# megaease/easevoice-trainer

Measured on AMD Instinct MI355X. Metric: audio-seconds/sec trained (s2), higher is better.
Workload: dtype bf16; 1 GPU; s2 SoVITS generator+discriminator GAN step, batch=16/GPU, 4 s 32 kHz clips (T=200 frames), configs/s2.json, random-init weights; global_batch=16, parallelism=dp1, launch=hip-graph replay (3 graphs/step)

## Files before the change

### easevoice_trainer_amd/csrc/elementwise.hip

```cpp
#include "evt_common.h"
#include "../../include/evt.h"

namespace {

__device__ __forceinline__ void store_w(void* base, long idx, float w, int dtype) {
  if (dtype == EVT_DT_HALF) reinterpret_cast<h16_t*>(base)[idx] = f2h(w);
  else reinterpret_cast<float*>(base)[idx] = w;
}

__device__ __forceinline__ long reg_idx(const evt_wlayout& L, int d0, int d1, int kk) {
  const int chunk = d1 / L.reg_ck, cc = d1 - chunk * L.reg_ck;
  return (((long)d0 * L.reg_nchunk + chunk) * L.reg_kp + kk) * L.reg_ck + cc;
}

__device__ __forceinline__ long alt_idx(const evt_wlayout& L, int d0, int d1, int kk) {
  const int chunk = d0 / L.alt_ck, cc = d0 - chunk * L.alt_ck;
  if (L.stride == 1) {
    const int t = L.k - 1 - kk;
    return (((long)d1 * L.alt_nchunk + chunk) * L.alt_kp + t) * L.alt_ck + cc;
  }
  const int J = (L.k + L.stride - 1) / L.stride;
  const int ph = kk % L.stride, j = kk / L.stride;
  const int jp = J - 1 - j;
  return ((((long)ph * L.d1 + d1) * L.alt_nchunk + chunk) * L.alt_kp + jp) * L.alt_ck + cc;
// ... 360 lines not shown

constexpr int SEG_MAX = 64;

template <typename T, int MODE>
__device__ __forceinline__ float seg_term(float a, float b, float target) {
  if (MODE == 0) return fabsf(a - b);
  const float d = target - a;
  return d * d;
}
template <typename T, int MODE>
__device__ __forceinline__ float seg_grad(float a, float b, float target, float dl) {
  if (MODE == 0) { const float d = a - b; return d > 0.f ? dl : (d < 0.f ? -dl : 0.f); }
  return -2.f * (target - a) * dl;
}

template <typename T, int MODE, bool BWD>
__global__ __launch_bounds__(256) void seg_flat_kernel(const evt_seg* segs, int nseg, float target, float* out,
                                                       const float* dloss) {
  constexpr int V = 16 / sizeof(T);
  __shared__ float red[4];
  __shared__ long pre[SEG_MAX + 1];
  if (threadIdx.x == 0) {
    long acc = 0;
    for (int i = 0; i < nseg; ++i) { pre[i] = acc; acc += segs[i].n; }
    pre[nseg] = acc;
  }
  __syncthreads();
  const long total = pre[nseg];
  long chunk = (total + gridDim.x - 1) / gridDim.x;
  chunk = (chunk + 2047) / 2048 * 2048;
  const long lo = (long)blockIdx.x * chunk, hi = min(total, lo + chunk);
  float acc = 0.f;
  for (int si = 0; si < nseg; ++si) {
    const long s0 = pre[si], s1 = pre[si + 1];
    if (s1 <= lo || s0 >= hi) continue;
    const evt_seg s = segs[si];
    if (BWD && !s.da) continue;
    const T* a = reinterpret_cast<const T*>(s.a);
    const T* b = reinterpret_cast<const T*>(s.b);
    T* da = reinterpret_cast<T*>(s.da);
    const long i0 = max(lo, s0) - s0, i1 = min(hi, s1) - s0;
    const float dl = BWD ? dloss[0] * s.scale : 0.f;
    float part = 0.f;
    const long v0 = min(i1, (i0 + V - 1) / V * V), v1 = v0 + (i1 - v0) / V * V;
    const bool vec_ok = ((((uintptr_t)a) | (MODE == 0 ? (uintptr_t)b : 0) | (BWD ? (uintptr_t)da : 0)) & 15) == 0;
    if (vec_ok) {
      for (long i = i0 + threadIdx.x; i < v0; i += 256) {
        const float av = to_f<T>(a[i]), bv = MODE == 0 ? to_f<T>(b[i]) : 0.f;
        if (BWD) da[i] = from_f<T>(seg_grad<T, MODE>(av, bv, target, dl)); else part += seg_term<T, MODE>(av, bv, target);
      }
      for (long i = v0 + (long)threadIdx.x * V; i < v1; i += 256L * V) {
        const uint4 va = *reinterpret_cast<const uint4*>(a + i);
        uint4 vb = make_uint4(0, 0, 0, 0);
        if (MODE == 0) vb = *reinterpret_cast<const uint4*>(b + i);
        const T* pa = reinterpret_cast<const T*>(&va);
        const T* pb = reinterpret_cast<const T*>(&vb);
        uint4 vo;
        T* po = reinterpret_cast<T*>(&vo);
#pragma unroll
        for (int e = 0; e < V; ++e) {
          const float av = to_f<T>(pa[e]), bv = MODE == 0 ? to_f<T>(pb[e]) : 0.f;
          if (BWD) po[e] = from_f<T>(seg_grad<T, MODE>(av, bv, target, dl)); else part += seg_term<T, MODE>(av, bv, target);
        }
        if (BWD) *reinterpret_cast<uint4*>(da + i) = vo;
      }
      for (long i = v1 + threadIdx.x; i < i1; i += 256) {
        const float av = to_f<T>(a[i]), bv = MODE == 0 ? to_f<T>(b[i]) : 0.f;
        if (BWD) da[i] = from_f<T>(seg_grad<T, MODE>(av, bv, target, dl)); else part += seg_term<T, MODE>(av, bv, target);
      }
    } else {
      for (long i = i0 + threadIdx.x; i < i1; i += 256) {
        const float av = to_f<T>(a[i]), bv = MODE == 0 ? to_f<T>(b[i]) : 0.f;
        if (BWD) da[i] = from_f<T>(seg_grad<T, MODE>(av, bv, target, dl)); else part += seg_term<T, MODE>(av, bv, target);
      }
    }
    acc += part * s.scale;
  }
  if (!BWD) {
    acc = block_reduce_sum_256(acc, red);
    if (threadIdx.x == 0 && acc != 0.f) atomicAdd(out, acc);
  }
}

__global__ void adamw_flat_kernel(float* p, const float* g, float* m, float* v, const evt_adamw_seg* segs, int nseg,
                                  float b1, float b2, float eps, float bc1, float bc2_sqrt, float gscale,
                                  long lo, long hi) {
  for (long i = lo + blockIdx.x * (long)blockDim.x + threadIdx.x; i < hi; i += (long)gridDim.x * blockDim.x) {
    int si = -1;
// ... 375 lines not shown
```

### easevoice_trainer_amd/csrc/losses.hip

```cpp
#include "evt_common.h"
#include "../../include/evt.h"

namespace {

__device__ __forceinline__ float ld_any(const void* p, int dt, long i) {
  return dt == EVT_DT_HALF ? h2f(reinterpret_cast<const h16_t*>(p)[i]) : reinterpret_cast<const float*>(p)[i];
}
__device__ __forceinline__ void st_any(void* p, int dt, long i, float v) {
  if (dt == EVT_DT_HALF) reinterpret_cast<h16_t*>(p)[i] = f2h(v); else reinterpret_cast<float*>(p)[i] = v;
}

struct KlArgs {
  const void* zp; const void* lq; const void* mp; const void* lp;
  void* dzp; void* dlq; void* dmp; void* dlp;
  int dt_zp, dt_lq, dt_mp, dt_lp;
  const int* lens;
  int B, T, C, time_inner;
};

__device__ __forceinline__ bool kl_live(const KlArgs& a, long i) {
  if (!a.lens) return true;
  long b, t;
  if (a.time_inner) { t = i % a.T; b = i / ((long)a.T * a.C); }
  else { const long row = i / a.C; b = row / a.T; t = row - b * a.T; }
  return t < a.lens[b];
}

__global__ __launch_bounds__(256) void masked_kl_fwd_kernel(KlArgs a, long n, float* out) {
  __shared__ float red[4];
  float acc = 0.f;
  for (long i = blockIdx.x * 256L + threadIdx.x; i < n; i += (long)gridDim.x * 256) {
    if (!kl_live(a, i)) continue;
    const float zp = ld_any(a.zp, a.dt_zp, i), lq = ld_any(a.lq, a.dt_lq, i), mp = ld_any(a.mp, a.dt_mp, i),
                lp = ld_any(a.lp, a.dt_lp, i);
    const float d = zp - mp;
    acc += lp - lq - 0.5f + 0.5f * d * d * __expf(-2.f * lp);
  }
  acc = block_reduce_sum_256(acc, red);
  if (threadIdx.x == 0) atomicAdd(out, acc);
  if (blockIdx.x == 0 && threadIdx.x == 0) {
    long cnt = 0;
    for (int b = 0; b < a.B; ++b) cnt += a.lens ? min(max(a.lens[b], 0), a.T) : a.T;
    out[1] = (float)cnt;
  }
}

__global__ __launch_bounds__(256) void masked_kl_bwd_kernel(KlArgs a, long n, const float* dloss, const float* count) {
  const float g = dloss[0] / count[0];
  for (long i = blockIdx.x * 256L + threadIdx.x; i < n; i += (long)gridDim.x * 256) {
    float gz = 0.f, glq = 0.f, glp = 0.f;
    if (kl_live(a, i)) {
      const float zp = ld_any(a.zp, a.dt_zp, i), mp = ld_any(a.mp, a.dt_mp, i), lp = ld_any(a.lp, a.dt_lp, i);
      const float d = zp - mp, e = __expf(-2.f * lp);
      gz = g * d * e;
      glq = -g;
      glp = g * (1.f - d * d * e);
    }
    if (a.dzp) st_any(a.dzp, a.dt_zp, i, gz);
    if (a.dlq) st_any(a.dlq, a.dt_lq, i, glq);
    if (a.dmp) st_any(a.dmp, a.dt_mp, i, -gz);
    if (a.dlp) st_any(a.dlp, a.dt_lp, i, glp);
  }
}

int kl_args(KlArgs& a, const evt_kl_params* p, const void* zp, const void* lq, const void* mp, const void* lp,
            const int32_t* lens) {
  if (!p || !zp || !lq || !mp || !lp || p->B <= 0 || p->T <= 0 || p->C <= 0) return EVT_EINVAL;
  const int dts[4] = {p->dt_z_p, p->dt_logs_q, p->dt_m_p, p->dt_logs_p};
  for (int d : dts) if (d != EVT_DT_F32 && d != EVT_DT_HALF) return EVT_EINVAL;
  a.zp = zp; a.lq = lq; a.mp = mp; a.lp = lp;
  a.dzp = a.dlq = a.dmp = a.dlp = nullptr;
  a.dt_zp = dts[0]; a.dt_lq = dts[1]; a.dt_mp = dts[2]; a.dt_lp = dts[3];
  a.lens = lens; a.B = p->B; a.T = p->T; a.C = p->C; a.time_inner = p->time_inner ? 1 : 0;
  return EVT_OK;
}

}

extern "C" {

int evt_masked_kl_fwd(const evt_kl_params* p, const void* z_p, const void* logs_q, const void* m_p, const void* logs_p,
                      const int32_t* lens, float* out2, void* stream) {
  KlArgs a;
  if (int rc = kl_args(a, p, z_p, logs_q, m_p, logs_p, lens)) return rc;
  if (!out2) return EVT_EINVAL;
  const long n = (long)p->B * p->T * p->C;
  long blocks = (n + 256L * 8 - 1) / (256L * 8);
  if (blocks > 2048) blocks = 2048;
  hipLaunchKernelGGL(masked_kl_fwd_kernel, dim3((unsigned)blocks), dim3(256), 0, (hipStream_t)stream, a, n, out2);
  return evt_check_launch();
}

int evt_masked_kl_bwd(const evt_kl_params* p, const void* z_p, const void* logs_q, const void* m_p, const void* logs_p,
                      const int32_t* lens, const float* dloss, const float* count, void* dz_p, void* dlogs_q, void* dm_p,
                      void* dlogs_p, void* stream) {
  KlArgs a;
  if (int rc = kl_args(a, p, z_p, logs_q, m_p, logs_p, lens)) return rc;
  if (!dloss || !count) return EVT_EINVAL;
  a.dzp = dz_p; a.dlq = dlogs_q; a.dmp = dm_p; a.dlp = dlogs_p;
  const long n = (long)p->B * p->T * p->C;
  long blocks = (n + 256L * 8 - 1) / (256L * 8);
  if (blocks > 2048) blocks = 2048;
  hipLaunchKernelGGL(masked_kl_bwd_kernel, dim3((unsigned)blocks), dim3(256), 0, (hipStream_t)stream, a, n, dloss, count);
  return evt_check_launch();
}

int64_t evt_workspace_bytes(int32_t op, const int64_t* dims, int32_t ndims) {
  if (!dims && ndims > 0) return -1;
  switch (op) {
    case EVT_WS_MEL:
      if (ndims != 5) return -1;
      return 4 * evt_mel_workspace_floats((int32_t)dims[0], (int32_t)dims[1], (int32_t)dims[2], (int32_t)dims[3],
                                          (int32_t)dims[4]);
    case EVT_WS_ATTN_BWD:
    case EVT_WS_MHA_BWD:
      if (ndims != 3) return -1;
      return 4 * dims[0] * dims[1] * dims[2];
    case EVT_WS_MASKED_KL:
// ... 10 lines not shown
```

### easevoice_trainer_amd/hip/disc.py

```python
import ctypes as C
import os

import torch

from . import conv as HC
from . import lib as L

_ALL = os.environ.get("EVT_BRANCH_STREAMS", "1") != "0"
MPD_STREAMS = int(os.environ.get("EVT_MPD_STREAMS", "2")) if _ALL else 1
_side = {}


def _new_stream(dev, k):
    return L.role_stream(dev, f"lane{k}", ring=1)


def _branches(dev, n_items):
    n = MPD_STREAMS if (dev.type == "cuda" and HC.TRACE is None) else 1
    if n <= 1:
        return [None] * n_items, []
    pool = _side.setdefault(dev, [])
    while len(pool) < n - 1:
        pool.append(_new_stream(dev, len(pool)))
    lanes = [None] + pool[: n - 1]
# ... 69 lines not shown
    @staticmethod
    def forward(ctx, x, periods, cd):
        ctx.periods, ctx.shape, ctx.dtype = periods, tuple(x.shape), x.dtype
        return tuple(mpd_fold(periods, cd, x))

    @staticmethod
    def backward(ctx, *grads):
        n, T = ctx.shape
        gs = []
        for g, p in zip(grads, ctx.periods):
            gs.append(g if g is not None else torch.zeros((n * p, (T + p - 1) // p, 1), dtype=grads[0].dtype,
                                                          device=grads[0].device))
        return mpd_unfold(ctx.periods, gs, 0, n, T, ctx.dtype), None, None


def _seg_table(a, b, da, scales, device):
    segs = [L.Seg(x.data_ptr(), y.data_ptr() if y is not None else None, g.data_ptr() if g is not None else None,
                  x.numel(), sc, 0) for x, y, g, sc in zip(a, b, da, scales)]
    return L.struct_to_device(segs, device)


class MPDGenLossFn(torch.autograd.Function):
    @staticmethod
    def forward(ctx, anchor, plan, periods, y_hat, y_real):
        nd = len(plan)
        n_items, T = y_hat.shape
        dev = y_hat.device
        cd = plan[0][0][0].bank.dtype
        dt = L.dt_code(cd)
        both = mpd_fold(periods, cd, y_real, y_hat)
        maps, saved = [], []
        lanes, sides = _branches(dev, nd)
        main = torch.cuda.current_stream(dev) if sides else None
# ... 21 lines not shown
            lg = ys[-1][ys[-1].size(0) // 2:]
            la.append(lg)
            ls.append(1.0 / lg.numel())
        out = torch.zeros(2, dtype=torch.float32, device=dev)
        L.check(L.lib().evt_l1_multi_fwd(dt, L.ptr(_seg_table(fa, fb, [None] * len(fa), fs, dev)), len(fa),
                                         L.ptr(out[1:]), L.stream_ptr()), "evt_l1_multi_fwd")
        L.check(L.lib().evt_lsgan_multi_fwd(dt, L.ptr(_seg_table(la, [None] * nd, [None] * nd, ls, dev)), nd,
                                            1.0, L.ptr(out[:1]), L.stream_ptr()), "evt_lsgan_multi_fwd")
        ctx.plan, ctx.dt = plan, dt
        ctx.counts = [len(ys) for ys in maps]
        ctx.in_shapes = [(x.size(0) // 2, x.size(1), 1) for x in both]
        ctx.periods, ctx.wav = periods, (n_items, T, y_hat.dtype)
        ctx.save_for_backward(*[y for ys in maps for y in ys])
        logits = [lg.reshape(n_items, -1).detach() for lg in la]
        ctx.mark_non_differentiable(*logits)
        return (out[0], out[1], *logits)

    @staticmethod
    def backward(ctx, dgen, dfm, *_unused):
        plan, dt = ctx.plan, ctx.dt
        flat = list(ctx.saved_tensors)
        maps, at = [], 0
        for c in ctx.counts:
            maps.append(flat[at: at + c])
            at += c
        dev = flat[0].device
        nd = len(plan)
        fa, fb, fs, fg, la, ls, lgr = [], [], [], [], [], [], []
        for ys in maps:
            for y in ys:
                h = y.size(0) // 2
                fa.append(y[h:])
                fb.append(y[:h])
                fs.append(2.0 / y[h:].numel())
                fg.append(torch.empty_like(y[h:]))
            lg = ys[-1][ys[-1].size(0) // 2:]
            la.append(lg)
            ls.append(1.0 / lg.numel())
            lgr.append(torch.empty_like(lg))
        dl = torch.stack([dgen.reshape(()).float(), dfm.reshape(()).float()]).contiguous()
        L.check(L.lib().evt_l1_multi_bwd(dt, L.ptr(_seg_table(fa, fb, fg, fs, dev)), len(fa), L.ptr(dl[1:]),
                                         L.stream_ptr()), "evt_l1_multi_bwd")
        L.check(L.lib().evt_lsgan_multi_bwd(dt, L.ptr(_seg_table(la, [None] * nd, lgr, ls, dev)), nd, 1.0,
                                            L.ptr(dl[:1]), L.stream_ptr()), "evt_lsgan_multi_bwd")
        grads, gi = [], 0
        lanes, sides = _branches(dev, nd)
        main = torch.cuda.current_stream(dev) if sides else None
        for st in sides:
            st.wait_stream(main)
        for (slots, acts), ys, lg_grad, in_shape, lane in zip(plan, maps, lgr, ctx.in_shapes, lanes):
            nl = len(slots)
            mg = fg[gi: gi + nl]
            gi += nl
            with _On(lane):
                dy = _branch_bwd(slots, acts, ys, mg, lg_grad, in_shape, dt)
            if lane is not None:
                dy.record_stream(main)
            grads.append(dy)
        for st in sides:
            main.wait_stream(st)
        n_items, T, wdt = ctx.wav
        return None, None, None, mpd_unfold(ctx.periods, grads, 0, n_items, T, wdt), None


def _branch_bwd(slots, acts, ys, mg, lg_grad, in_shape, dt):
    nl = len(slots)
    dy = mg[-1] + lg_grad
    for l in reversed(range(nl)):
        s, (act, slope) = slots[l], acts[l]
        y_act = ys[l][ys[l].size(0) // 2:]
        half = y_act.size(0)
        lin = ys[l - 1].size(1) if l > 0 else in_shape[1]
        add = mg[l - 1] if l > 0 else None
        a_kind, a_slope, y_arg = act, slope, (y_act if act != L.ACT_NONE else None)
        if act != L.ACT_NONE and L.lib().evt_conv1d_wants_plain_dy(C.byref(s.params(half, lin, 1.0, act, slope))):
            dy_eff = torch.empty_like(dy)
            L.check(L.lib().evt_dact_mul(dt, L.ptr(dy), L.ptr(y_act), int(act), float(slope), L.ptr(dy_eff),
                                         dy.numel(), L.stream_ptr()), "evt_dact_mul")
            dy, y_arg, a_kind, a_slope = dy_eff, None, L.ACT_NONE, 1.0
        dy = HC._bwd_data(s, dy.contiguous(), y_arg, None, add, half, lin, 1.0, a_kind, a_slope)
    return dy
```

### easevoice_trainer_amd/hip/lib.py

```python
import ctypes as C
import os
import re

import torch

from ..build import HEADER

_HERE = os.path.dirname(os.path.abspath(__file__))
LIB_PATH = os.path.join(os.path.dirname(_HERE), "libevt_hip.so")
LIB_PATH_F16 = os.path.join(os.path.dirname(_HERE), "libevt_hip_f16.so")

DT_F32, DT_BF16, DT_F16 = 0, 1, 2
HALF_DTYPES = (torch.bfloat16, torch.float16)
ACT_NONE, ACT_LRELU, ACT_TANH = 0, 1, 2
IMPL_AUTO, IMPL_NAIVE, IMPL_IGEMM = 0, 1, 2


class EvtError(RuntimeError):
    pass


EVT_OK, EVT_ELAUNCH, EVT_EINVAL, EVT_ENOTSUP = 0, 5, 22, 95


# ... 54 lines not shown
class WgradMember(C.Structure):
    _fields_ = [("p", C.c_void_p), ("x", C.c_void_p), ("dy", C.c_void_p), ("y", C.c_void_p), ("dw", C.c_void_p),
                ("dbias", C.c_void_p), ("sp", C.c_void_p)]


class WgradPlan(C.Structure):
    _fields_ = [("tiles", C.c_int64), ("stages", C.c_int32), ("min_stages", C.c_int32), ("parts", C.c_int32),
                ("launch", C.c_int32), ("nsplit", C.c_int32), ("per", C.c_int32)]


WGRAD_GROUP_MAX = 16


class Seg(C.Structure):
    _fields_ = [("a", C.c_void_p), ("b", C.c_void_p), ("da", C.c_void_p), ("n", C.c_int64),
                ("scale", C.c_float), ("pad_", C.c_int32)]


class KlParams(C.Structure):
    _fields_ = [("B", C.c_int32), ("T", C.c_int32), ("C", C.c_int32), ("time_inner", C.c_int32),
                ("dt_z_p", C.c_int32), ("dt_logs_q", C.c_int32), ("dt_m_p", C.c_int32), ("dt_logs_p", C.c_int32)]


class AdamWSeg(C.Structure):
    _fields_ = [("begin", C.c_int64), ("end", C.c_int64), ("lr", C.c_float), ("weight_decay", C.c_float)]


class AttnParams(C.Structure):
    _fields_ = [
        ("dtype", C.c_int32), ("B", C.c_int32), ("L", C.c_int32), ("H", C.c_int32), ("D", C.c_int32),
        ("x_len", C.c_int32),
        ("q_stride_b", C.c_int64), ("q_stride_l", C.c_int64), ("q_stride_h", C.c_int64),
        ("o_stride_b", C.c_int64), ("o_stride_l", C.c_int64), ("o_stride_h", C.c_int64),
        ("dropout_p", C.c_float), ("seed", C.c_uint32),
    ]

# ... 234 lines not shown
```

### easevoice_trainer_amd/module/commons.py

```python
import torch


def sequence_mask(length, max_length=None):
    if max_length is None:
        max_length = int(length.max())
    x = torch.arange(max_length, dtype=length.dtype, device=length.device)
    return x.unsqueeze(0) < length.unsqueeze(1)


def slice_segments(x, ids_str, segment_size=4):
    idx = ids_str.view(-1, 1) + torch.arange(segment_size, device=x.device).view(1, -1)
    return torch.gather(x, 1, idx.unsqueeze(-1).expand(-1, -1, x.size(2)))


def slice_segments_1d(x, ids_str, segment_size):
    idx = ids_str.view(-1, 1) + torch.arange(segment_size, device=x.device).view(1, -1)
    return torch.gather(x, 1, idx)


def rand_slice_segments(x, x_lengths=None, segment_size=4):
    b, t, _ = x.shape
    if x_lengths is None:
        x_lengths = torch.full((b,), t, device=x.device)
    ids_str_max = x_lengths - segment_size + 1
    ids_str = (torch.rand([b], device=x.device) * ids_str_max).to(dtype=torch.long)
    return slice_segments(x, ids_str, segment_size), ids_str
```

### easevoice_trainer_amd/module/losses.py

```python
import ctypes as C

import torch

from ..hip import lib as L


def _table(pairs, scales, grads, device):
    segs = []
    for (a, b), sc, da in zip(pairs, scales, grads):
        segs.append(L.Seg(a.data_ptr(), b.data_ptr() if b is not None else None,
                          da.data_ptr() if da is not None else None, a.numel(), sc, 0))
    return L.struct_to_device(segs, device)


class _SegLossFn(torch.autograd.Function):

    @staticmethod
    def forward(ctx, mode, target, scales, n_a, *tensors):
        a_list, b_list = tensors[:n_a], tensors[n_a:]
        a_list = [t.contiguous() for t in a_list]
        b_list = [t.contiguous() for t in b_list] if mode == 0 else [None] * n_a
        dev = a_list[0].device
        dt = L.dt_of(a_list[0])
        out = torch.zeros(1, dtype=torch.float32, device=dev)
# ... 98 lines not shown
        T, Cc = (d2, d1) if time_inner else (d1, d2)
        prm = L.KlParams(B, T, Cc, int(time_inner), *[L.dt_of(t) for t in ts])
        out2 = torch.zeros(2, dtype=torch.float32, device=z_p.device)
        L.check(L.lib().evt_masked_kl_fwd(C.byref(prm), *[L.ptr(t) for t in ts], L.ptr(lens), L.ptr(out2),
                                          L.stream_ptr()), "evt_masked_kl_fwd")
        ctx.save_for_backward(z_p, logs_q, m_p, logs_p, lens, out2)
        ctx.prm = prm
        return out2[0] / out2[1]

    @staticmethod
    def backward(ctx, dloss):
        z_p, logs_q, m_p, logs_p, lens, out2 = ctx.saved_tensors
        ts = (z_p, logs_q, m_p, logs_p)
        grads = [torch.empty_like(t) if ctx.needs_input_grad[i] else None for i, t in enumerate(ts)]
        dl = dloss.reshape(1).float().contiguous()
        L.check(L.lib().evt_masked_kl_bwd(C.byref(ctx.prm), *[L.ptr(t) for t in ts], L.ptr(lens), L.ptr(dl),
                                          L.ptr(out2[1:]), *[L.ptr(g) for g in grads], L.stream_ptr()),
                "evt_masked_kl_bwd")
        return (*grads, None, None)


def kl_loss(z_p, logs_q, m_p, logs_p, z_mask, lens=None):
    ts = [z_p, logs_q, m_p, logs_p]
    if z_mask.dim() != 3 or z_mask.size(1) != 1 or any(t.dim() != 3 or t.shape != z_p.shape for t in ts) \
            or z_mask.size(-1) != z_p.size(-1) or z_mask.size(0) != z_p.size(0):
        raise L.EvtError(f"kl_loss: [B, C, T] tensors and a [B, 1, T] mask expected, got {[tuple(t.shape) for t in ts]} "
                         f"/ {tuple(z_mask.shape)}")
    if lens is None:
        lens = z_mask.reshape(z_mask.size(0), -1).sum(1)
    lens = lens.to(torch.int32).contiguous()
    B, Cc, T = z_p.shape
    if T > 1 and Cc > 1 and all(t.stride() == (T * Cc, 1, Cc) for t in ts):
        return _MaskedKLFn.apply(*[t.transpose(1, 2) for t in ts], lens, False)
    return _MaskedKLFn.apply(*[t.contiguous() for t in ts], lens, True)
```

### easevoice_trainer_amd/train/s2_engine.py

```python
import os
from dataclasses import dataclass, field
from types import SimpleNamespace
from typing import Optional

import torch
from torch.nn import functional as F

from ..hip import lib as L
from ..hip.enc import bump_rng
from ..module import commons
from ..module.losses import (discriminator_loss, discriminator_loss_batched, feature_loss, generator_loss, kl_loss,
                             l1_mean_scaled)
from ..module.mel_processing import mel_spectrogram_torch, spec_to_mel_slices
from ..module.models import MultiPeriodDiscriminator, SynthesizerTrn
from ..runtime import DeviceGradScaler, FlatAdamW, ModelRuntime


@dataclass
class S2Losses:
    disc: torch.Tensor
    gen: torch.Tensor
    fm: torch.Tensor
    mel: torch.Tensor
    kl: torch.Tensor
    kl_ssl: torch.Tensor
    gen_all: torch.Tensor
    grad_sumsq_d: Optional[torch.Tensor] = None
# ... 87 lines not shown
        if lane is not None:
            main = torch.cuda.current_stream(self.device)
            lane.wait_stream(main)
            with torch.cuda.stream(lane):
                st.y_mel = spec_to_mel_slices(st.spec, st.ids_slice, seg // hop, d["filter_length"], d["n_mel_channels"],
                                              d["sampling_rate"], d["mel_fmin"], d["mel_fmax"])
                st.y_hat_mel = mel_spectrogram_torch(st.y_hat.squeeze(1), d["filter_length"], d["n_mel_channels"],
                                                     d["sampling_rate"], hop, d["win_length"], d["mel_fmin"], d["mel_fmax"])
            for t in (st.spec, st.ids_slice, st.y_hat):
                t.record_stream(lane)
        else:
            st.y_mel = spec_to_mel_slices(st.spec, st.ids_slice, seg // hop, d["filter_length"], d["n_mel_channels"],
                                          d["sampling_rate"], d["mel_fmin"], d["mel_fmax"])
            st.y_hat_mel = mel_spectrogram_torch(st.y_hat.squeeze(1), d["filter_length"], d["n_mel_channels"],
                                                 d["sampling_rate"], hop, d["win_length"], d["mel_fmin"], d["mel_fmax"])
        st.y_seg = commons.slice_segments_1d(st.y.squeeze(1), st.ids_slice * hop, seg)
        rt_d.bank.weight_grads = True
        if self.device.type == "cuda":
            outs = net_d.forward_batched(st.y_seg, st.y_hat.detach())
            if not backward:
                st.d_losses = [discriminator_loss_batched([o]) for o in outs]
            else:
                st.loss_disc = discriminator_loss_batched(outs)
        else:
            y_d_hat_r, y_d_hat_g, _, _ = net_d(st.y_seg, st.y_hat.detach())
            if not backward:
                st.d_losses = [discriminator_loss([r], [g]) for r, g in zip(y_d_hat_r, y_d_hat_g)]
            else:
                st.loss_disc = discriminator_loss(y_d_hat_r, y_d_hat_g)
        if not backward:
            st.d_done = []
# ... 11 lines not shown
        net_d, rt_g, rt_d = self.net_d, self.rt_g, self.rt_d
        self.scaler.unscale_(rt_d)
        st.gss_d = rt_d.grad_sumsq() * (st.inv_world * st.inv_world)
        if st.hook_after_d is not None:
            st.hook_after_d()
        if st.do_opt and not getattr(st, "piped", False):
            self.optim_d.step(grad_scale=st.inv_world, **self._skip(rt_d))
            rt_d.prepare()
        rt_d.bank.weight_grads = False
        st.loss_gen, st.loss_fm, st.y_d_hat_g = net_d.generator_losses(st.y_seg, st.y_hat)
        z, z_p, m_p, logs_p, m_q, logs_q = st.lat
        if self.device.type == "cuda" and st.y_mel.dtype == st.y_hat_mel.dtype:
            st.loss_mel = l1_mean_scaled(st.y_hat_mel, st.y_mel, t["c_mel"])
        else:
            st.loss_mel = F.l1_loss(st.y_mel, st.y_hat_mel) * t["c_mel"]
        st.loss_kl = kl_loss(z_p, logs_q, m_p, logs_p, st.z_mask, lens=st.spec_lengths) * t["c_kl"]
        st.loss_gen_all = st.loss_gen + st.loss_fm + st.loss_mel + st.kl_ssl * 1 + st.loss_kl
        if not backward:
            return
        self.scaler.scale(st.loss_gen_all).backward()
        rt_d.bank.weight_grads = True
        rt_g.finish_grads()

    def _skip(self, rt):
        return dict(skip=self.scaler.found_inf(rt)) if self.scaler.enabled else {}

    def _phase_c(self, st):
        self.scaler.unscale_(self.rt_g)
        st.gss_g = self.rt_g.grad_sumsq() * (st.inv_world * st.inv_world)
        if st.do_opt:
            self.optim_g.step(grad_scale=st.inv_world, **self._skip(self.rt_g))
            self.scaler.update()
# ... 286 lines not shown
```

### include/evt.h

```cpp
#ifndef EVT_H
#define EVT_H
#include <stddef.h>
#include <stdint.h>

#ifdef __cplusplus
extern "C" {
#endif
#pragma GCC visibility push(default)

#define EVT_DT_F32 0
#define EVT_DT_BF16 1
#define EVT_DT_F16 2
#define EVT_ACT_NONE 0
#define EVT_ACT_LRELU 1
#define EVT_ACT_TANH 2
#define EVT_IMPL_AUTO 0
#define EVT_IMPL_NAIVE 1
#define EVT_IMPL_IGEMM 2

const char* evt_version(void);
int32_t evt_half_dtype(void);
void evt_debug_kernel_tags(int32_t enable);
const char* evt_last_kernel_tag(void);

// ... 189 lines not shown
                float* dwav, int32_t nseq, int32_t wav_len, int32_t n_fft, int32_t hop, int32_t n_mels, void* stream);
int64_t evt_mel_workspace_floats(int32_t nseq, int32_t wav_len, int32_t n_fft, int32_t hop, int32_t n_mels);

int evt_ref_spec_rows(const float* x, const int32_t* lens, int32_t nseq, int32_t N, const float* window, int32_t n_fft,
                      int32_t hop, int32_t bins, float* out, float* peak, void* stream);

int evt_ncl_to_nlc(int32_t dtype, const float* src, void* dst, int32_t B, int32_t C, int32_t T, int32_t Cp, void* stream);

int evt_rvq_norms(const float* embed, float* ee, int32_t K, int32_t D, void* stream);
int evt_rvq_select(const float* h, const float* dots, const float* embed, const float* ee, int64_t* codes, float* q_out,
                   int32_t N, int32_t D, int32_t K, int32_t rep, void* stream);

int evt_spec_to_mel(const float* spec, const float* basis, const int64_t* starts, float* out, int32_t B, int32_t F,
                    int32_t T, int32_t M, int32_t nfr, void* stream);

typedef struct evt_seg { const void* a; const void* b; void* da; int64_t n; float scale; int32_t pad_; } evt_seg;
int evt_l1_multi_fwd(int32_t dtype, const evt_seg* segs, int32_t nseg, float* out, void* stream);
int evt_l1_multi_bwd(int32_t dtype, const evt_seg* segs, int32_t nseg, const float* dloss, void* stream);
int evt_lsgan_multi_fwd(int32_t dtype, const evt_seg* segs, int32_t nseg, float target, float* out, void* stream);
int evt_lsgan_multi_bwd(int32_t dtype, const evt_seg* segs, int32_t nseg, float target, const float* dloss,
                        void* stream);

typedef struct evt_kl_params {
  int32_t B, T, C, time_inner;
  int32_t dt_z_p, dt_logs_q, dt_m_p, dt_logs_p;
} evt_kl_params;
int evt_masked_kl_fwd(const evt_kl_params* p, const void* z_p, const void* logs_q, const void* m_p, const void* logs_p,
                      const int32_t* lens, float* out2, void* stream);
int evt_masked_kl_bwd(const evt_kl_params* p, const void* z_p, const void* logs_q, const void* m_p, const void* logs_p,
                      const int32_t* lens, const float* dloss, const float* count, void* dz_p, void* dlogs_q, void* dm_p,
                      void* dlogs_p, void* stream);

typedef struct evt_adamw_seg { int64_t begin, end; float lr; float weight_decay; } evt_adamw_seg;
int evt_adamw_flat(float* param, const float* grad, float* exp_avg, float* exp_avg_sq, int64_t n,
                   const evt_adamw_seg* segs, int32_t nseg, float beta1, float beta2, float eps, int32_t step,
                   float grad_scale, void* stream);
int evt_adamw_flat_dev(float* param, const float* grad, float* exp_avg, float* exp_avg_sq, int64_t n,
                       const evt_adamw_seg* segs, int32_t nseg, float beta1, float beta2, float eps,
                       int32_t* step_counter, float grad_scale, void* stream);
int evt_adamw_flat_dev_range(float* param, const float* grad, float* exp_avg, float* exp_avg_sq, int64_t lo, int64_t hi,
                             const evt_adamw_seg* segs, int32_t nseg, float beta1, float beta2, float eps,
                             int32_t* step_counter, int32_t bump, float grad_scale, void* stream);
int evt_mpd_fold(int32_t src0_dtype, const void* src0, int32_t n0, int32_t src1_dtype, const void* src1, int32_t n1, int32_t T,
                 const int32_t* periods, int32_t nper, void* const* outs, int32_t out_dtype, void* stream);
int evt_mpd_unfold(int32_t grad_dtype, const void* const* douts, const int32_t* periods, int32_t nper, int32_t b0, int32_t n,
                   int32_t T, int32_t dsrc_dtype, void* dsrc, void* stream);
// ... 261 lines not shown
```

Baseline: 3564 audio-s/s.

## Fuse generator loss total with KL, accumulate LSGAN grads in place, add slice kernels

Adds a fused generator-total path. The masked KL is computed on strided operands without a contiguous copy, and a single tiny kernel sums the loss terms, with the c_kl scale folded into the KL backward. The LSGAN backward now accumulates straight into the feature-map gradient buffer instead of writing a separate tensor that is added later. New slice-rows forward and backward kernels replace generic segment slicing. Together these remove several small elementwise launches and copies per step, at the cost of extra read-modify-write in the grad kernel and more custom code paths.

```diff
diff --git a/easevoice_trainer_amd/csrc/elementwise.hip b/easevoice_trainer_amd/csrc/elementwise.hip
--- a/easevoice_trainer_amd/csrc/elementwise.hip
+++ b/easevoice_trainer_amd/csrc/elementwise.hip
@@ -398,6 +398,15 @@
   return -2.f * (target - a) * dl;
 }
 
+template <typename T>
+__device__ __forceinline__ T seg_out(T old, float g, bool acc) {
+  const T r = from_f<T>(g);
+  if (!acc) return r;
+  float rf = to_f<T>(r);
+  asm volatile("" : "+v"(rf));
+  return from_f<T>(to_f<T>(old) + rf);
+}
+
 template <typename T, int MODE, bool BWD>
 __global__ __launch_bounds__(256) void seg_flat_kernel(const evt_seg* segs, int nseg, float target, float* out,
                                                        const float* dloss) {
@@ -425,13 +434,14 @@
     T* da = reinterpret_cast<T*>(s.da);
     const long i0 = max(lo, s0) - s0, i1 = min(hi, s1) - s0;
     const float dl = BWD ? dloss[0] * s.scale : 0.f;
+    const bool acc_da = BWD && s.accum != 0;
     float part = 0.f;
     const long v0 = min(i1, (i0 + V - 1) / V * V), v1 = v0 + (i1 - v0) / V * V;
     const bool vec_ok = ((((uintptr_t)a) | (MODE == 0 ? (uintptr_t)b : 0) | (BWD ? (uintptr_t)da : 0)) & 15) == 0;
     if (vec_ok) {
       for (long i = i0 + threadIdx.x; i < v0; i += 256) {
         const float av = to_f<T>(a[i]), bv = MODE == 0 ? to_f<T>(b[i]) : 0.f;
-        if (BWD) da[i] = from_f<T>(seg_grad<T, MODE>(av, bv, target, dl)); else part += seg_term<T, MODE>(av, bv, target);
+        if (BWD) da[i] = seg_out<T>(da[i], seg_grad<T, MODE>(av, bv, target, dl), acc_da); else part += seg_term<T, MODE>(av, bv, target);
       }
       for (long i = v0 + (long)threadIdx.x * V; i < v1; i += 256L * V) {
         const uint4 va = *reinterpret_cast<const uint4*>(a + i);
@@ -439,23 +449,24 @@
         if (MODE == 0) vb = *reinterpret_cast<const uint4*>(b + i);
         const T* pa = reinterpret_cast<const T*>(&va);
         const T* pb = reinterpret_cast<const T*>(&vb);
-        uint4 vo;
+        uint4 vo = make_uint4(0, 0, 0, 0);
+        if (BWD && acc_da) vo = *reinterpret_cast<const uint4*>(da + i);
         T* po = reinterpret_cast<T*>(&vo);
 #pragma unroll
         for (int e = 0; e < V; ++e) {
           const float av = to_f<T>(pa[e]), bv = MODE == 0 ? to_f<T>(pb[e]) : 0.f;
-          if (BWD) po[e] = from_f<T>(seg_grad<T, MODE>(av, bv, target, dl)); else part += seg_term<T, MODE>(av, bv, target);
+          if (BWD) po[e] = seg_out<T>(po[e], seg_grad<T, MODE>(av, bv, target, dl), acc_da); else part += seg_term<T, MODE>(av, bv, target);
         }
         if (BWD) *reinterpret_cast<uint4*>(da + i) = vo;
       }
       for (long i = v1 + threadIdx.x; i < i1; i += 256) {
         const float av = to_f<T>(a[i]), bv = MODE == 0 ? to_f<T>(b[i]) : 0.f;
-        if (BWD) da[i] = from_f<T>(seg_grad<T, MODE>(av, bv, target, dl)); else part += seg_term<T, MODE>(av, bv, target);
+        if (BWD) da[i] = seg_out<T>(da[i], seg_grad<T, MODE>(av, bv, target, dl), acc_da); else part += seg_term<T, MODE>(av, bv, target);
       }
     } else {
       for (long i = i0 + threadIdx.x; i < i1; i += 256) {
         const float av = to_f<T>(a[i]), bv = MODE == 0 ? to_f<T>(b[i]) : 0.f;
-        if (BWD) da[i] = from_f<T>(seg_grad<T, MODE>(av, bv, target, dl)); else part += seg_term<T, MODE>(av, bv, target);
+        if (BWD) da[i] = seg_out<T>(da[i], seg_grad<T, MODE>(av, bv, target, dl), acc_da); else part += seg_term<T, MODE>(av, bv, target);
       }
     }
     acc += part * s.scale;
diff --git a/easevoice_trainer_amd/csrc/losses.hip b/easevoice_trainer_amd/csrc/losses.hip
--- a/easevoice_trainer_amd/csrc/losses.hip
+++ b/easevoice_trainer_amd/csrc/losses.hip
@@ -16,7 +16,14 @@
   int dt_zp, dt_lq, dt_mp, dt_lp;
   const int* lens;
   int B, T, C, time_inner;
+  int ld_zp, ld_lq, ld_mp, ld_lp;
 };
+
+__device__ __forceinline__ long kl_at(const KlArgs& a, long i, int ld) {
+  if (a.time_inner || ld == a.C) return i;
+  const long row = i / a.C;
+  return row * ld + (i - row * a.C);
+}
 
 __device__ __forceinline__ bool kl_live(const KlArgs& a, long i) {
   if (!a.lens) return true;
@@ -31,8 +38,8 @@
   float acc = 0.f;
   for (long i = blockIdx.x * 256L + threadIdx.x; i < n; i += (long)gridDim.x * 256) {
     if (!kl_live(a, i)) continue;
-    const float zp = ld_any(a.zp, a.dt_zp, i), lq = ld_any(a.lq, a.dt_lq, i), mp = ld_any(a.mp, a.dt_mp, i),
-                lp = ld_any(a.lp, a.dt_lp, i);
+    const float zp = ld_any(a.zp, a.dt_zp, kl_at(a, i, a.ld_zp)), lq = ld_any(a.lq, a.dt_lq, kl_at(a, i, a.ld_lq)),
+                mp = ld_any(a.mp, a.dt_mp, kl_at(a, i, a.ld_mp)), lp = ld_any(a.lp, a.dt_lp, kl_at(a, i, a.ld_lp));
     const float d = zp - mp;
     acc += lp - lq - 0.5f + 0.5f * d * d * __expf(-2.f * lp);
   }
@@ -45,12 +52,14 @@
   }
 }
 
-__global__ __launch_bounds__(256) void masked_kl_bwd_kernel(KlArgs a, long n, const float* dloss, const float* count) {
-  const float g = dloss[0] / count[0];
+__global__ __launch_bounds__(256) void masked_kl_bwd_kernel(KlArgs a, long n, const float* dloss, float scale,
+                                                            const float* count) {
+  const float g = __fmul_rn(dloss[0], scale) / count[0];
   for (long i = blockIdx.x * 256L + threadIdx.x; i < n; i += (long)gridDim.x * 256) {
     float gz = 0.f, glq = 0.f, glp = 0.f;
     if (kl_live(a, i)) {
-      const float zp = ld_any(a.zp, a.dt_zp, i), mp = ld_any(a.mp, a.dt_mp, i), lp = ld_any(a.lp, a.dt_lp, i);
+      const float zp = ld_any(a.zp, a.dt_zp, kl_at(a, i, a.ld_zp)), mp = ld_any(a.mp, a.dt_mp, kl_at(a, i, a.ld_mp)),
+                  lp = ld_any(a.lp, a.dt_lp, kl_at(a, i, a.ld_lp));
       const float d = zp - mp, e = __expf(-2.f * lp);
       gz = g * d * e;
       glq = -g;
@@ -63,6 +72,17 @@
   }
 }
 
+__global__ void gen_total_kernel(const float* gen, const float* fm, const float* mel, const float* kl_ssl, const float* kl2,
+                                 float c_kl, float* out2) {
+#pragma clang fp contract(off)
+  const float kl = __fmul_rn(__fdiv_rn(kl2[0], kl2[1]), c_kl);
+  float s = __fadd_rn(gen[0], fm[0]);
+  s = __fadd_rn(s, mel[0]);
+  s = __fadd_rn(s, __fmul_rn(kl_ssl[0], 1.f));
+  out2[0] = __fadd_rn(s, kl);
+  out2[1] = kl;
+}
+
 int kl_args(KlArgs& a, const evt_kl_params* p, const void* zp, const void* lq, const void* mp, const void* lp,
             const int32_t* lens) {
   if (!p || !zp || !lq || !mp || !lp || p->B <= 0 || p->T <= 0 || p->C <= 0) return EVT_EINVAL;
@@ -72,6 +92,10 @@
   a.dzp = a.dlq = a.dmp = a.dlp = nullptr;
   a.dt_zp = dts[0]; a.dt_lq = dts[1]; a.dt_mp = dts[2]; a.dt_lp = dts[3];
   a.lens = lens; a.B = p->B; a.T = p->T; a.C = p->C; a.time_inner = p->time_inner ? 1 : 0;
+  const int lds[4] = {p->ld_z_p, p->ld_logs_q, p->ld_m_p, p->ld_logs_p};
+  for (int ld : lds) if (ld != 0 && (ld < p->C || (a.time_inner && ld != p->C))) return EVT_EINVAL;
+  a.ld_zp = lds[0] ? lds[0] : p->C; a.ld_lq = lds[1] ? lds[1] : p->C;
+  a.ld_mp = lds[2] ? lds[2] : p->C; a.ld_lp = lds[3] ? lds[3] : p->C;
   return EVT_OK;
 }
 
@@ -92,8 +116,8 @@
 }
 
 int evt_masked_kl_bwd(const evt_kl_params* p, const void* z_p, const void* logs_q, const void* m_p, const void* logs_p,
-                      const int32_t* lens, const float* dloss, const float* count, void* dz_p, void* dlogs_q, void* dm_p,
-                      void* dlogs_p, void* stream) {
+                      const int32_t* lens, const float* dloss, float scale, const float* count, void* dz_p, void* dlogs_q,
+                      void* dm_p, void* dlogs_p, void* stream) {
   KlArgs a;
   if (int rc = kl_args(a, p, z_p, logs_q, m_p, logs_p, lens)) return rc;
   if (!dloss || !count) return EVT_EINVAL;
@@ -101,7 +125,16 @@
   const long n = (long)p->B * p->T * p->C;
   long blocks = (n + 256L * 8 - 1) / (256L * 8);
   if (blocks > 2048) blocks = 2048;
-  hipLaunchKernelGGL(masked_kl_bwd_kernel, dim3((unsigned)blocks), dim3(256), 0, (hipStream_t)stream, a, n, dloss, count);
+  hipLaunchKernelGGL(masked_kl_bwd_kernel, dim3((unsigned)blocks), dim3(256), 0, (hipStream_t)stream, a, n, dloss, scale,
+                     count);
+  return evt_check_launch();
+}
+
+int evt_gen_total_fwd(const float* loss_gen, const float* loss_fm, const float* loss_mel, const float* kl_ssl,
+                      const float* kl2, float c_kl, float* out2, void* stream) {
+  if (!loss_gen || !loss_fm || !loss_mel || !kl_ssl || !kl2 || !out2) return EVT_EINVAL;
+  hipLaunchKernelGGL(gen_total_kernel, dim3(1), dim3(1), 0, (hipStream_t)stream, loss_gen, loss_fm, loss_mel, kl_ssl, kl2,
+                     c_kl, out2);
   return evt_check_launch();
 }
 
diff --git a/easevoice_trainer_amd/csrc/seg_ops.hip b/easevoice_trainer_amd/csrc/seg_ops.hip
--- /dev/null
+++ b/easevoice_trainer_amd/csrc/seg_ops.hip
@@ -0,0 +1,115 @@
+#include "evt_common.h"
+#include "../../include/evt.h"
+
+namespace {
+
+__device__ __forceinline__ long seg_start(const int64_t* ids, int mul, const float* u, const int64_t* lens, int L, int seg,
+                                          int b) {
+  if (!u) return (long)ids[b] * mul;
+  const long n = lens ? (long)lens[b] : (long)L;
+  return (long)__fmul_rn(u[b], (float)(n - seg + 1));
+}
+
+__global__ __launch_bounds__(256) void slice_rows_fwd_kernel(const char* x, const int64_t* ids, int mul, const float* u,
+                                                             const int64_t* lens, int64_t* ids_out, int L, int seg,
+                                                             long row_bytes, char* y) {
+  const int b = blockIdx.y;
+  const long start = seg_start(ids, mul, u, lens, L, seg, b);
+  if (ids_out && blockIdx.x == 0 && threadIdx.x == 0) ids_out[b] = start;
+  const long nbytes = (long)seg * row_bytes;
+  const long off0 = start * row_bytes, lim = (long)L * row_bytes;
+  const char* src = x + (long)b * lim;
+  char* dst = y + (long)b * nbytes;
+  const bool vec = (((uintptr_t)(src + off0) | (uintptr_t)dst | (uintptr_t)nbytes) & 15) == 0;
+  if (vec) {
+    const long nv = nbytes >> 4;
+    for (long v = blockIdx.x * 256L + threadIdx.x; v < nv; v += (long)gridDim.x * 256) {
+      const long o = off0 + (v << 4);
+      uint4 val = make_uint4(0, 0, 0, 0);
+      if (o >= 0 && o + 16 <= lim) {
+        val = *reinterpret_cast<const uint4*>(src + o);
+      } else {
+        char* pv = reinterpret_cast<char*>(&val);
+        for (int e = 0; e < 16; ++e)
+          if (o + e >= 0 && o + e < lim) pv[e] = src[o + e];
+      }
+      *reinterpret_cast<uint4*>(dst + (v << 4)) = val;
+    }
+  } else {
+    for (long j = blockIdx.x * 256L + threadIdx.x; j < nbytes; j += (long)gridDim.x * 256) {
+      const long o = off0 + j;
+      dst[j] = (o >= 0 && o < lim) ? src[o] : (char)0;
+    }
+  }
+}
+
+template <typename T>
+__global__ __launch_bounds__(256) void slice_rows_bwd_kernel(const T* dy, const int64_t* ids, int mul, int L, int seg, int C,
+                                                             T* dx) {
+  constexpr int V = 16 / sizeof(T);
+  const int b = blockIdx.y;
+  const long start = (long)ids[b] * mul;
+  const long n = (long)L * C;
+  const T* src = dy + (long)b * seg * C;
+  T* dst = dx + (long)b * n;
+  const bool vec = C % V == 0 && (((uintptr_t)dy | (uintptr_t)dx) & 15) == 0;
+  if (vec) {
+    const long nv = n / V;
+    for (long v = blockIdx.x * 256L + threadIdx.x; v < nv; v += (long)gridDim.x * 256) {
+      const long e0 = v * V;
+      const long s = e0 / C - start;
+      uint4 val = make_uint4(0, 0, 0, 0);
+      if (s >= 0 && s < seg) {
+        val = *reinterpret_cast<const uint4*>(src + s * C + e0 % C);
+        T* pv = reinterpret_cast<T*>(&val);
+#pragma unroll
+        for (int e = 0; e < V; ++e) pv[e] = from_f<T>(0.f + to_f<T>(pv[e]));
+      }
+      *reinterpret_cast<uint4*>(dst + e0) = val;
+    }
+  } else {
+    for (long i = blockIdx.x * 256L + threadIdx.x; i < n; i += (long)gridDim.x * 256) {
+      const long s = i / C - start;
+      dst[i] = (s >= 0 && s < seg) ? from_f<T>(0.f + to_f<T>(src[s * C + i % C])) : from_f<T>(0.f);
+    }
+  }
+}
+
+inline unsigned blocks_for(long items) {
+  long b = (items + 255) / 256;
+  if (b > 1024) b = 1024;
+  if (b < 1) b = 1;
+  return (unsigned)b;
+}
+
+}
+
+extern "C" {
+
+int evt_slice_rows_fwd(const void* x, const int64_t* ids, int32_t mul, const float* u, const int64_t* lens, int64_t* ids_out,
+                       int32_t nseq, int32_t L, int32_t seg, int64_t row_bytes, void* y, void* stream) {
+  if (!x || !y || (!ids && !u) || (ids && u) || nseq <= 0 || nseq > 65535 || L <= 0 || seg <= 0 || row_bytes <= 0)
+    return EVT_EINVAL;
+  if (u && !ids_out) return EVT_EINVAL;
+  const long nbytes = (long)seg * row_bytes;
+  hipLaunchKernelGGL(slice_rows_fwd_kernel, dim3(blocks_for(nbytes >> 4), nseq), dim3(256), 0, (hipStream_t)stream,
+                     (const char*)x, ids, (int)(u ? 1 : mul), u, lens, ids_out, (int)L, (int)seg, (long)row_bytes, (char*)y);
+  return evt_check_launch();
+}
+
+int evt_slice_rows_bwd(int32_t dtype, const void* dy, const int64_t* ids, int32_t mul, int32_t nseq, int32_t L, int32_t seg,
+                       int32_t C, void* dx, void* stream) {
+  if (!dy || !ids || !dx || nseq <= 0 || nseq > 65535 || L <= 0 || seg <= 0 || C <= 0) return EVT_EINVAL;
+  hipStream_t st = (hipStream_t)stream;
+  const long n = (long)L * C;
+  if (dtype == EVT_DT_HALF)
+    hipLaunchKernelGGL(slice_rows_bwd_kernel<h16_t>, dim3(blocks_for(n / 8), nseq), dim3(256), 0, st, (const h16_t*)dy, ids,
+                       (int)mul, (int)L, (int)seg, (int)C, (h16_t*)dx);
+  else if (dtype == EVT_DT_F32)
+    hipLaunchKernelGGL(slice_rows_bwd_kernel<float>, dim3(blocks_for(n / 4), nseq), dim3(256), 0, st, (const float*)dy, ids,
+                       (int)mul, (int)L, (int)seg, (int)C, (float*)dx);
+  else return EVT_EINVAL;
+  return evt_check_launch();
+}
+
+}
diff --git a/easevoice_trainer_amd/hip/disc.py b/easevoice_trainer_amd/hip/disc.py
--- a/easevoice_trainer_amd/hip/disc.py
+++ b/easevoice_trainer_amd/hip/disc.py
@@ -107,9 +107,9 @@
         return mpd_unfold(ctx.periods, gs, 0, n, T, ctx.dtype), None, None
 
 
-def _seg_table(a, b, da, scales, device):
+def _seg_table(a, b, da, scales, device, accum=0):
     segs = [L.Seg(x.data_ptr(), y.data_ptr() if y is not None else None, g.data_ptr() if g is not None else None,
-                  x.numel(), sc, 0) for x, y, g, sc in zip(a, b, da, scales)]
+                  x.numel(), sc, accum) for x, y, g, sc in zip(a, b, da, scales)]
     return L.struct_to_device(segs, device)
 
 
@@ -161,6 +161,7 @@
         ctx.save_for_backward(*[y for ys in maps for y in ys])
         logits = [lg.reshape(n_items, -1).detach() for lg in la]
         ctx.mark_non_differentiable(*logits)
+        ctx.set_materialize_grads(False)
         return (out[0], out[1], *logits)
 
     @staticmethod
@@ -184,23 +185,25 @@
             lg = ys[-1][ys[-1].size(0) // 2:]
             la.append(lg)
             ls.append(1.0 / lg.numel())
-            lgr.append(torch.empty_like(lg))
-        dl = torch.stack([dgen.reshape(()).float(), dfm.reshape(()).float()]).contiguous()
+            lgr.append(fg[-1])
+        zero = lambda: torch.zeros((), dtype=torch.float32, device=dev)
+        dl = torch.stack([dgen.reshape(()).float() if dgen is not None else zero(),
+                          dfm.reshape(()).float() if dfm is not None else zero()]).contiguous()
         L.check(L.lib().evt_l1_multi_bwd(dt, L.ptr(_seg_table(fa, fb, fg, fs, dev)), len(fa), L.ptr(dl[1:]),
                                          L.stream_ptr()), "evt_l1_multi_bwd")
-        L.check(L.lib().evt_lsgan_multi_bwd(dt, L.ptr(_seg_table(la, [None] * nd, lgr, ls, dev)), nd, 1.0,
+        L.check(L.lib().evt_lsgan_multi_bwd(dt, L.ptr(_seg_table(la, [None] * nd, lgr, ls, dev, accum=1)), nd, 1.0,
                                             L.ptr(dl[:1]), L.stream_ptr()), "evt_lsgan_multi_bwd")
         grads, gi = [], 0
         lanes, sides = _branches(dev, nd)
         main = torch.cuda.current_stream(dev) if sides else None
         for st in sides:
             st.wait_stream(main)
-        for (slots, acts), ys, lg_grad, in_shape, lane in zip(plan, maps, lgr, ctx.in_shapes, lanes):
+        for (slots, acts), ys, in_shape, lane in zip(plan, maps, ctx.in_shapes, lanes):
             nl = len(slots)
             mg = fg[gi: gi + nl]
             gi += nl
             with _On(lane):
-                dy = _branch_bwd(slots, acts, ys, mg, lg_grad, in_shape, dt)
+                dy = _branch_bwd(slots, acts, ys, mg, in_shape, dt)
             if lane is not None:
                 dy.record_stream(main)
             grads.append(dy)
@@ -210,9 +213,9 @@
         return None, None, None, mpd_unfold(ctx.periods, grads, 0, n_items, T, wdt), None
 
 
-def _branch_bwd(slots, acts, ys, mg, lg_grad, in_shape, dt):
+def _branch_bwd(slots, acts, ys, mg, in_shape, dt):
     nl = len(slots)
-    dy = mg[-1] + lg_grad
+    dy = mg[-1]
     for l in reversed(range(nl)):
         s, (act, slope) = slots[l], acts[l]
         y_act = ys[l][ys[l].size(0) // 2:]
diff --git a/easevoice_trainer_amd/hip/lib.py b/easevoice_trainer_amd/hip/lib.py
--- a/easevoice_trainer_amd/hip/lib.py
+++ b/easevoice_trainer_amd/hip/lib.py
@@ -92,12 +92,13 @@
 
 class Seg(C.Structure):
     _fields_ = [("a", C.c_void_p), ("b", C.c_void_p), ("da", C.c_void_p), ("n", C.c_int64),
-                ("scale", C.c_float), ("pad_", C.c_int32)]
+                ("scale", C.c_float), ("accum", C.c_int32)]
 
 
 class KlParams(C.Structure):
     _fields_ = [("B", C.c_int32), ("T", C.c_int32), ("C", C.c_int32), ("time_inner", C.c_int32),
-                ("dt_z_p", C.c_int32), ("dt_logs_q", C.c_int32), ("dt_m_p", C.c_int32), ("dt_logs_p", C.c_int32)]
+                ("dt_z_p", C.c_int32), ("dt_logs_q", C.c_int32), ("dt_m_p", C.c_int32), ("dt_logs_p", C.c_int32),
+                ("ld_z_p", C.c_int32), ("ld_logs_q", C.c_int32), ("ld_m_p", C.c_int32), ("ld_logs_p", C.c_int32)]
 
 
 class AdamWSeg(C.Structure):
diff --git a/easevoice_trainer_amd/module/commons.py b/easevoice_trainer_amd/module/commons.py
--- a/easevoice_trainer_amd/module/commons.py
+++ b/easevoice_trainer_amd/module/commons.py
@@ -8,18 +8,65 @@
     return x.unsqueeze(0) < length.unsqueeze(1)
 
 
+class _SliceRowsFn(torch.autograd.Function):
+
+    @staticmethod
+    def forward(ctx, x, ids, mul, u, lens, seg):
+        from ..hip import lib as L
+
+        x = x.contiguous()
+        B, T = x.size(0), x.size(1)
+        row = x[0, 0].numel()
+        y = torch.empty((B, seg, *x.shape[2:]), dtype=x.dtype, device=x.device)
+        ids_out = None
+        if ids is None:
+            u = u.float().contiguous()
+            lens = lens.to(torch.long).contiguous() if lens is not None else None
+            ids_out = torch.empty(B, dtype=torch.long, device=x.device)
+        else:
+            ids = ids.to(torch.long).contiguous()
+        L.check(L.lib().evt_slice_rows_fwd(L.ptr(x), L.ptr(ids), int(mul), L.ptr(u), L.ptr(lens), L.ptr(ids_out), B, T,
+                                           int(seg), row * x.element_size(), L.ptr(y), L.stream_ptr()),
+                "evt_slice_rows_fwd")
+        starts = ids if ids is not None else ids_out
+        ctx.save_for_backward(starts)
+        ctx.geom = (B, T, int(seg), row, int(mul) if ids is not None else 1, x.shape, x.dtype)
+        if ids_out is None:
+            return y
+        ctx.mark_non_differentiable(ids_out)
+        return y, ids_out
+
+    @staticmethod
+    def backward(ctx, dy, *_unused):
+        from ..hip import lib as L
+
+        starts, = ctx.saved_tensors
+        B, T, seg, row, mul, shape, dtype = ctx.geom
+        dy = dy.contiguous()
+        dx = torch.empty(shape, dtype=dtype, device=dy.device)
+        L.check(L.lib().evt_slice_rows_bwd(L.dt_code(dtype), L.ptr(dy), L.ptr(starts), mul, B, T, seg, row, L.ptr(dx),
+                                           L.stream_ptr()), "evt_slice_rows_bwd")
+        return dx, None, None, None, None, None
+
+
 def slice_segments(x, ids_str, segment_size=4):
+    if x.is_cuda:
+        return _SliceRowsFn.apply(x, ids_str, 1, None, None, segment_size)
     idx = ids_str.view(-1, 1) + torch.arange(segment_size, device=x.device).view(1, -1)
     return torch.gather(x, 1, idx.unsqueeze(-1).expand(-1, -1, x.size(2)))
 
 
-def slice_segments_1d(x, ids_str, segment_size):
-    idx = ids_str.view(-1, 1) + torch.arange(segment_size, device=x.device).view(1, -1)
+def slice_segments_1d(x, ids_str, segment_size, mul=1):
+    if x.is_cuda:
+        return _SliceRowsFn.apply(x, ids_str, mul, None, None, segment_size)
+    idx = (ids_str * mul).view(-1, 1) + torch.arange(segment_size, device=x.device).view(1, -1)
     return torch.gather(x, 1, idx)
 
 
 def rand_slice_segments(x, x_lengths=None, segment_size=4):
     b, t, _ = x.shape
+    if x.is_cuda:
+        return _SliceRowsFn.apply(x, None, 1, torch.rand([b], device=x.device), x_lengths, segment_size)
     if x_lengths is None:
         x_lengths = torch.full((b,), t, device=x.device)
     ids_str_max = x_lengths - segment_size + 1
diff --git a/easevoice_trainer_amd/module/losses.py b/easevoice_trainer_amd/module/losses.py
--- a/easevoice_trainer_amd/module/losses.py
+++ b/easevoice_trainer_amd/module/losses.py
@@ -136,13 +136,56 @@
         ts = (z_p, logs_q, m_p, logs_p)
         grads = [torch.empty_like(t) if ctx.needs_input_grad[i] else None for i, t in enumerate(ts)]
         dl = dloss.reshape(1).float().contiguous()
-        L.check(L.lib().evt_masked_kl_bwd(C.byref(ctx.prm), *[L.ptr(t) for t in ts], L.ptr(lens), L.ptr(dl),
+        L.check(L.lib().evt_masked_kl_bwd(C.byref(ctx.prm), *[L.ptr(t) for t in ts], L.ptr(lens), L.ptr(dl), 1.0,
                                           L.ptr(out2[1:]), *[L.ptr(g) for g in grads], L.stream_ptr()),
                 "evt_masked_kl_bwd")
         return (*grads, None, None)
 
 
-def kl_loss(z_p, logs_q, m_p, logs_p, z_mask, lens=None):
+class _GenTotalFn(torch.autograd.Function):
+
+    @staticmethod
+    def forward(ctx, loss_gen, loss_fm, loss_mel, kl_ssl, z_p, logs_q, m_p, logs_p, lens, time_inner, c_kl, lds):
+        ts = (z_p, logs_q, m_p, logs_p)
+        terms = (loss_gen, loss_fm, loss_mel, kl_ssl)
+        B, d1, d2 = z_p.shape
+        T, Cc = (d2, d1) if time_inner else (d1, d2)
+        if any(t.shape != z_p.shape or ld < d2 or (time_inner and ld != d2) or t.stride(2) != 1 or t.stride(1) != ld
+               or (B > 1 and t.stride(0) != d1 * ld) for t, ld in zip(ts, lds)):
+            raise L.EvtError("gen_total: four tensors of one shape, rows contiguous and lds[i] elements apart, expected")
+        if any(t.numel() != 1 or t.dtype != torch.float32 or t.device != z_p.device for t in terms):
+            raise L.EvtError("gen_total: loss_gen, loss_fm, loss_mel and kl_ssl are fp32 scalars on the device of the KL tensors")
+        prm = L.KlParams(B, T, Cc, int(time_inner), *[L.dt_of(t) for t in ts], *([0] * 4 if time_inner else lds))
+        ptrs = [C.c_void_p(t.data_ptr()) for t in ts]
+        kl2 = torch.zeros(2, dtype=torch.float32, device=z_p.device)
+        L.check(L.lib().evt_masked_kl_fwd(C.byref(prm), ptrs[0], ptrs[1], ptrs[2], ptrs[3], L.ptr(lens), L.ptr(kl2),
+                                          L.stream_ptr()), "evt_masked_kl_fwd")
+        out = torch.empty(2, dtype=torch.float32, device=z_p.device)
+        L.check(L.lib().evt_gen_total_fwd(L.ptr(loss_gen), L.ptr(loss_fm), L.ptr(loss_mel), L.ptr(kl_ssl), L.ptr(kl2),
+                                          float(c_kl), L.ptr(out), L.stream_ptr()), "evt_gen_total_fwd")
+        ctx.save_for_backward(z_p, logs_q, m_p, logs_p, lens, kl2)
+        ctx.prm, ctx.c_kl = prm, float(c_kl)
+        ctx.set_materialize_grads(False)
+        total, loss_kl = out[0], out[1]
+        ctx.mark_non_differentiable(loss_kl)
+        return total, loss_kl
+
+    @staticmethod
+    def backward(ctx, dloss, _dkl):
+        z_p, logs_q, m_p, logs_p, lens, kl2 = ctx.saved_tensors
+        ts = (z_p, logs_q, m_p, logs_p)
+        grads = [torch.empty(t.shape, dtype=t.dtype, device=t.device) if ctx.needs_input_grad[4 + i] else None
+                 for i, t in enumerate(ts)]
+        dl = dloss.reshape(1).float().contiguous()
+        if any(g is not None for g in grads):
+            gz, gq, gm, gp = [L.ptr(g) for g in grads]
+            pz, pq, pm, pp = [C.c_void_p(t.data_ptr()) for t in ts]
+            L.check(L.lib().evt_masked_kl_bwd(C.byref(ctx.prm), pz, pq, pm, pp, L.ptr(lens), L.ptr(dl), ctx.c_kl,
+                                              L.ptr(kl2[1:]), gz, gq, gm, gp, L.stream_ptr()), "evt_masked_kl_bwd")
+        return (*[dloss if ctx.needs_input_grad[i] else None for i in range(4)], *grads, None, None, None, None)
+
+
+def _kl_operands(z_p, logs_q, m_p, logs_p, z_mask, lens, strided=False):
     ts = [z_p, logs_q, m_p, logs_p]
     if z_mask.dim() != 3 or z_mask.size(1) != 1 or any(t.dim() != 3 or t.shape != z_p.shape for t in ts) \
             or z_mask.size(-1) != z_p.size(-1) or z_mask.size(0) != z_p.size(0):
@@ -152,6 +195,19 @@
         lens = z_mask.reshape(z_mask.size(0), -1).sum(1)
     lens = lens.to(torch.int32).contiguous()
     B, Cc, T = z_p.shape
+    if strided and T > 1 and Cc > 1 and all(t.stride(1) == 1 and t.stride(2) >= Cc and t.stride(0) == T * t.stride(2)
+                                            for t in ts):
+        return [t.transpose(1, 2) for t in ts], lens, False, [t.stride(2) for t in ts]
     if T > 1 and Cc > 1 and all(t.stride() == (T * Cc, 1, Cc) for t in ts):
-        return _MaskedKLFn.apply(*[t.transpose(1, 2) for t in ts], lens, False)
-    return _MaskedKLFn.apply(*[t.contiguous() for t in ts], lens, True)
+        return ([t.transpose(1, 2) for t in ts], lens, False) + (([Cc] * 4,) if strided else ())
+    return ([t.contiguous() for t in ts], lens, True) + (([T] * 4,) if strided else ())
+
+
+def gen_total(loss_gen, loss_fm, loss_mel, kl_ssl, z_p, logs_q, m_p, logs_p, z_mask, c_kl, lens=None):
+    ts, lens, time_inner, lds = _kl_operands(z_p, logs_q, m_p, logs_p, z_mask, lens, strided=True)
+    return _GenTotalFn.apply(loss_gen, loss_fm, loss_mel, kl_ssl, *ts, lens, time_inner, c_kl, tuple(lds))
+
+
+def kl_loss(z_p, logs_q, m_p, logs_p, z_mask, lens=None):
+    ts, lens, time_inner = _kl_operands(z_p, logs_q, m_p, logs_p, z_mask, lens)
+    return _MaskedKLFn.apply(*ts, lens, time_inner)
diff --git a/easevoice_trainer_amd/train/s2_engine.py b/easevoice_trainer_amd/train/s2_engine.py
--- a/easevoice_trainer_amd/train/s2_engine.py
+++ b/easevoice_trainer_amd/train/s2_engine.py
@@ -9,8 +9,8 @@
 from ..hip import lib as L
 from ..hip.enc import bump_rng
 from ..module import commons
-from ..module.losses import (discriminator_loss, discriminator_loss_batched, feature_loss, generator_loss, kl_loss,
-                             l1_mean_scaled)
+from ..module.losses import (discriminator_loss, discriminator_loss_batched, feature_loss, gen_total, generator_loss,
+                             kl_loss, l1_mean_scaled)
 from ..module.mel_processing import mel_spectrogram_torch, spec_to_mel_slices
 from ..module.models import MultiPeriodDiscriminator, SynthesizerTrn
 from ..runtime import DeviceGradScaler, FlatAdamW, ModelRuntime
@@ -128,7 +128,7 @@
                                           d["sampling_rate"], d["mel_fmin"], d["mel_fmax"])
             st.y_hat_mel = mel_spectrogram_torch(st.y_hat.squeeze(1), d["filter_length"], d["n_mel_channels"],
                                                  d["sampling_rate"], hop, d["win_length"], d["mel_fmin"], d["mel_fmax"])
-        st.y_seg = commons.slice_segments_1d(st.y.squeeze(1), st.ids_slice * hop, seg)
+        st.y_seg = commons.slice_segments_1d(st.y.squeeze(1), st.ids_slice, seg, mul=hop)
         rt_d.bank.weight_grads = True
         if self.device.type == "cuda":
             outs = net_d.forward_batched(st.y_seg, st.y_hat.detach())
@@ -170,8 +170,12 @@
             st.loss_mel = l1_mean_scaled(st.y_hat_mel, st.y_mel, t["c_mel"])
         else:
             st.loss_mel = F.l1_loss(st.y_mel, st.y_hat_mel) * t["c_mel"]
-        st.loss_kl = kl_loss(z_p, logs_q, m_p, logs_p, st.z_mask, lens=st.spec_lengths) * t["c_kl"]
-        st.loss_gen_all = st.loss_gen + st.loss_fm + st.loss_mel + st.kl_ssl * 1 + st.loss_kl
+        if self.device.type == "cuda" and backward:
+            st.loss_gen_all, st.loss_kl = gen_total(st.loss_gen, st.loss_fm, st.loss_mel, st.kl_ssl, z_p, logs_q, m_p,
+                                                    logs_p, st.z_mask, t["c_kl"], lens=st.spec_lengths)
+        else:
+            st.loss_kl = kl_loss(z_p, logs_q, m_p, logs_p, st.z_mask, lens=st.spec_lengths) * t["c_kl"]
+            st.loss_gen_all = st.loss_gen + st.loss_fm + st.loss_mel + st.kl_ssl * 1 + st.loss_kl
         if not backward:
             return
         self.scaler.scale(st.loss_gen_all).backward()
diff --git a/include/evt.h b/include/evt.h
--- a/include/evt.h
+++ b/include/evt.h
@@ -227,7 +227,7 @@
 int evt_spec_to_mel(const float* spec, const float* basis, const int64_t* starts, float* out, int32_t B, int32_t F,
                     int32_t T, int32_t M, int32_t nfr, void* stream);
 
-typedef struct evt_seg { const void* a; const void* b; void* da; int64_t n; float scale; int32_t pad_; } evt_seg;
+typedef struct evt_seg { const void* a; const void* b; void* da; int64_t n; float scale; int32_t accum; } evt_seg;
 int evt_l1_multi_fwd(int32_t dtype, const evt_seg* segs, int32_t nseg, float* out, void* stream);
 int evt_l1_multi_bwd(int32_t dtype, const evt_seg* segs, int32_t nseg, const float* dloss, void* stream);
 int evt_lsgan_multi_fwd(int32_t dtype, const evt_seg* segs, int32_t nseg, float target, float* out, void* stream);
@@ -237,12 +237,20 @@
 typedef struct evt_kl_params {
   int32_t B, T, C, time_inner;
   int32_t dt_z_p, dt_logs_q, dt_m_p, dt_logs_p;
+  int32_t ld_z_p, ld_logs_q, ld_m_p, ld_logs_p;
 } evt_kl_params;
 int evt_masked_kl_fwd(const evt_kl_params* p, const void* z_p, const void* logs_q, const void* m_p, const void* logs_p,
                       const int32_t* lens, float* out2, void* stream);
 int evt_masked_kl_bwd(const evt_kl_params* p, const void* z_p, const void* logs_q, const void* m_p, const void* logs_p,
-                      const int32_t* lens, const float* dloss, const float* count, void* dz_p, void* dlogs_q, void* dm_p,
-                      void* dlogs_p, void* stream);
+                      const int32_t* lens, const float* dloss, float scale, const float* count, void* dz_p, void* dlogs_q,
+                      void* dm_p, void* dlogs_p, void* stream);
+int evt_gen_total_fwd(const float* loss_gen, const float* loss_fm, const float* loss_mel, const float* kl_ssl,
+                      const float* kl2, float c_kl, float* out2, void* stream);
+
+int evt_slice_rows_fwd(const void* x, const int64_t* ids, int32_t mul, const float* u, const int64_t* lens, int64_t* ids_out,
+                       int32_t nseq, int32_t L, int32_t seg, int64_t row_bytes, void* y, void* stream);
+int evt_slice_rows_bwd(int32_t dtype, const void* dy, const int64_t* ids, int32_t mul, int32_t nseq, int32_t L, int32_t seg,
+                       int32_t C, void* dx, void* stream);
 
 typedef struct evt_adamw_seg { int64_t begin, end; float lr; float weight_decay; } evt_adamw_seg;
 int evt_adamw_flat(float* param, const float* grad, float* exp_avg, float* exp_avg_sq, int64_t n,
```

After: 3588 audio-s/s (median of 6 runs). No clear change (+0.7%).
